# dnjulek/vapoursynth-zip

Hardware: AMD Instinct MI355X
Metric: frames/sec at 4K YUV420P16: Bilateral, BoxBlur, SSIMULACRA2 on 1/2/4/8 MI355X (higher is better)
Workload: dtype u16; 1 GPU; vszip.BoxBlur hradius=vradius=13, 3840x2160 YUV420P16, splitmix64 noise, HBM-resident; parallelism=frame-parallel x1, arena_candidates=5

## Files before the change

vapoursynth-zip_amd/csrc/boxblur_ct.hpp:

```cpp
#pragma once
#include <cmath>
#include <cstdlib>
#include <utility>

#include "plane_table.hpp"

namespace {

#ifndef VSZIP_ST_AUX
#define VSZIP_ST_AUX 2
#endif
#ifndef VSZIP_LD_AUX
#define VSZIP_LD_AUX 0
#endif
#ifndef VSZIP_ST8_AUX
#define VSZIP_ST8_AUX 0
#endif
#ifndef VSZIP_ST16_AUX
#define VSZIP_ST16_AUX 2
#endif
constexpr int kStoreAux = VSZIP_ST_AUX, kLoadAux = VSZIP_LD_AUX, kStoreAux8 = VSZIP_ST8_AUX, kStoreAux16 = VSZIP_ST16_AUX;
typedef uint32_t U32x4 __attribute__((ext_vector_type(4)));
typedef uint32_t U32x2 __attribute__((ext_vector_type(2)));

constexpr int kMaxPlanes = 48;
constexpr int PX = 8;

struct BBPlane {
    const void *src;
    void *dst;
    int sstride, dstride;
    int w, h;
    int block0;
    int ntx;
    int nbands;
    int nperiods;
    int cx0;
};

struct BBParams {
    BBPlane p[kMaxPlanes];
    int nplanes;
    int band_rows;
    int nblocks;
};

constexpr int kRingMaxPlanes = 192;
constexpr int kRingMaxBlocks = 8192;
struct RingParams {
    BBPlane p[kRingMaxPlanes];
    int nplanes;
    int nblocks;
    uint8_t plane_of_block[kRingMaxBlocks];
};

__device__ __forceinline__ int ct_tap_row(int k, int i, int radius, int ih) {
    const int dist_from_bottom = ih - 1 - i;
    if (k < radius) return (i < radius - k) ? min(radius - k - i, ih - 1) : (i - radius + k);
    return (dist_from_bottom < k - radius) ? (i - min(k - radius - dist_from_bottom, i)) : (i - radius + k);
}

template <typename T>
struct Raw8;
template <>
struct Raw8<uint16_t> {
    uint4 q;
};
template <>
struct Raw8<uint8_t> {
    uint2 q;
};

__device__ __forceinline__ void unpack8(const Raw8<uint16_t> &r, uint32_t v[PX]) {
    v[0] = r.q.x & 0xffffu; v[1] = r.q.x >> 16;
    v[2] = r.q.y & 0xffffu; v[3] = r.q.y >> 16;
    v[4] = r.q.z & 0xffffu; v[5] = r.q.z >> 16;
    v[6] = r.q.w & 0xffffu; v[7] = r.q.w >> 16;
}

__device__ __forceinline__ void unpack8(const Raw8<uint8_t> &r, uint32_t v[PX]) {
    v[0] = r.q.x & 0xffu; v[1] = (r.q.x >> 8) & 0xffu; v[2] = (r.q.x >> 16) & 0xffu; v[3] = r.q.x >> 24;
    v[4] = r.q.y & 0xffu; v[5] = (r.q.y >> 8) & 0xffu; v[6] = (r.q.y >> 16) & 0xffu; v[7] = r.q.y >> 24;
}

__device__ __forceinline__ void pack8(const uint32_t v[PX], Raw8<uint16_t> &r) {
    r.q.x = v[0] | (v[1] << 16);
    r.q.y = v[2] | (v[3] << 16);
    r.q.z = v[4] | (v[5] << 16);
    r.q.w = v[6] | (v[7] << 16);
// ... 133 lines not shown
    }

    const int ci = lane * PX;
#pragma unroll 1
    for (int i = y0; i < y1; ++i) {
        Raw8<T> an, sn;
        const bool more = i + 1 < y1;
        if (more) {
            const int n = i + 1;
            const int ar = (n + R < h) ? n + R : n - 1;
            const int sr = (n <= R) ? R - n + 1 : n - R - 1;
            an = load8<T>(src + (size_t)ar * pl.sstride, vx0, w, in_fast);
            sn = load8<T>(src + (size_t)sr * pl.sstride, vx0, w, in_fast);
        }

        uint32_t p[PX];
#pragma unroll
        for (int k = 0; k < PX; ++k) p[k] = __umulhi(col[k] + R, MAGIC);
#pragma unroll
        for (int k = 1; k < PX; ++k) p[k] += p[k - 1];
        const uint32_t incl = DPP ? wave_incl_scan_dpp(p[PX - 1]) : wave_incl_scan_shfl(p[PX - 1]);
        const uint32_t base = incl - p[PX - 1];
#pragma unroll
        for (int k = 0; k < PX; ++k) p[k] += base;
        *reinterpret_cast<uint4 *>(&P[ci]) = make_uint4(p[0], p[1], p[2], p[3]);
        *reinterpret_cast<uint4 *>(&P[ci + 4]) = make_uint4(p[4], p[5], p[6], p[7]);
        wave_lds_fence();

        if (is_out) {
            const uint32_t e0 = P[R] + P[R - 1];
            const uint32_t krow = 32768u + (uint32_t)(((uint64_t)e0 * INVLO) >> 16);
            uint32_t o[PX];
#pragma unroll
            for (int k = 0; k < PX; ++k) {
                const uint32_t e = P[ci + k + R] - P[ci + k - R - 1];
                o[k] = (uint32_t)(((uint64_t)e * INV2 + krow) >> 16);
            }
            store8<T>(dst + (size_t)i * pl.dstride, vx0, w, out_fast, o);
        }
        wave_lds_fence();

        if (more) {
            uint32_t a[PX], sb[PX];
            unpack8(an, a);
            unpack8(sn, sb);
#pragma unroll
            for (int k = 0; k < PX; ++k) col[k] += a[k] - sb[k];
        }
    }
}



template <int R, int SLOT_VGPRS = 4, int PXN = 8, int RV = R>
struct RingGeom {
    static constexpr int K = 2 * RV + 1;
    static constexpr int HL = ((R + 1 + PXN - 1) / PXN) * PXN;
    static constexpr int HR = ((R + PXN - 1) / PXN) * PXN;
#ifdef VSZIP_RING_OUT_LANES
    static constexpr int OUT_LANES = VSZIP_RING_OUT_LANES < 64 - HL / PXN - HR / PXN ? VSZIP_RING_OUT_LANES : 64 - HL / PXN - HR / PXN;
#else
    static constexpr int OUT_LANES = 64 - HL / PXN - HR / PXN;
#endif
    static constexpr int TWO = OUT_LANES * PXN;
    static constexpr int est_vgprs(int d) { return (2 * RV + 1 + d) * SLOT_VGPRS + (PXN == 16 ? 104 : 56); }
    static constexpr int tier(int v) { return v <= 128 ? 4 : (v <= 168 ? 3 : 2); }
    static constexpr int D3 = (2 * RV + 4) % 3 == 0 ? 3 : ((2 * RV + 6) % 3 == 0 ? 5 : 7);
#ifdef VSZIP_RING_D
    static constexpr int D = VSZIP_RING_D | 1;
    static constexpr int KL = (2 * RV + 1 + D) % 3 == 0 ? 3 : 2;
#else
    static constexpr bool SHALLOW = tier(est_vgprs(1)) > tier(est_vgprs(D3));
    static constexpr int D = SHALLOW ? 1 : D3;
    static constexpr int KL = SHALLOW ? 2 : 3;
#endif
    static constexpr int NR = 2 * RV + 1 + D;
#ifdef VSZIP_RING_WPE
    static constexpr int WPE = VSZIP_RING_WPE;
#else
    static constexpr int WPE = (SLOT_VGPRS == 2 && PXN == 8) ? (tier(est_vgprs(D)) > 3 ? 3 : tier(est_vgprs(D))) : tier(est_vgprs(D));
#endif
    static_assert(NR % KL == 0, "K-column ring must divide the period");
    static constexpr uint32_t MAGIC = K > 1 ? (uint32_t)(((1ull << 32) + K - 1) / K) : 0u;
};

template <typename T, int R, bool GENERAL, int PXN = 8, bool HONLY = false>
struct RingWave {
    static_assert(PXN == 8 || (PXN == 16 && sizeof(T) == 1 && !GENERAL), "16 pixels a lane: 8-bit planes, whole 16-pixel groups");
    static constexpr int RV = HONLY ? 0 : R;
    using G = RingGeom<R, (int)(sizeof(T) * PXN / 4), PXN, RV>;
    using RawT = RawN<T, PXN>;
    using Vec = decltype(RawT{}.q);
    static constexpr int NR = G::NR;
    static constexpr uint64_t INV = ((1ull << 32) + R) / (uint64_t)(2 * R + 1);
    static constexpr uint32_t INV2 = (uint32_t)(INV >> 16);

    RawT ring[NR];
    uint32_t col[PXN];
    uint32_t kcol;
    uint32_t kwgt;
    uint32_t kvo;
    uint32_t kn[G::KL], ko[G::KL];
    uint32_t kn_off, ko_off;
    uint32_t kr_prev;
    uint32_t *P;
    const char *srcb;
    char *dstb;
    uint32_t coff;
    uint32_t doff;
    uint32_t next_off;
    uint32_t out_off;
    uint32_t srow, drow;
    int w, h, lane, c0;
    bool rev, ld_ok, is_out, out_full;
    bool plain;
    __amdgpu_buffer_rsrc_t rs, rd;
    uint32_t sdoff;
    uint32_t psel;
    static constexpr uint32_t kOOB = 0xfffffff0u;

    __device__ __forceinline__ RawT fetch_off(uint32_t row_off) const {
        RawT t;
        if constexpr (sizeof(T) * PXN == 16) {
            const auto v = __builtin_amdgcn_raw_buffer_load_b128(rs, coff, row_off, sizeof(T) == 2 ? kLoadAux : 0);
            t.q = make_uint4(v[0], v[1], v[2], v[3]);
        } else {
            const auto v = __builtin_amdgcn_raw_buffer_load_b64(rs, coff, row_off, 0);
            t.q = make_uint2(v[0], v[1]);
        }
        return t;
    }
    __device__ __forceinline__ uint32_t fetch_px(uint32_t row_off) const {
        if constexpr (sizeof(T) == 2)
            return __builtin_amdgcn_raw_buffer_load_b16(rs, kvo, row_off, 0);
        else
            return __builtin_amdgcn_raw_buffer_load_b8(rs, kvo, row_off, 0);
    }
    __device__ __forceinline__ uint32_t krow_now() const {
        constexpr uint32_t INVLO = (uint32_t)(INV & 0xffffu);
        uint32_t v = __umul24(G::K > 1 ? __umulhi(kcol, G::MAGIC) : kcol, kwgt);
        v += (uint32_t)__builtin_amdgcn_update_dpp(0, (int)v, 0x111, 0xf, 0xf, false);
        v += (uint32_t)__builtin_amdgcn_update_dpp(0, (int)v, 0x112, 0xf, 0xf, false);
        v += (uint32_t)__builtin_amdgcn_update_dpp(0, (int)v, 0x114, 0xf, 0xf, false);
        v += (uint32_t)__builtin_amdgcn_update_dpp(0, (int)v, 0x118, 0xf, 0xf, false);
        uint32_t e0;
        if constexpr (R < 16) {
            e0 = (uint32_t)__builtin_amdgcn_readlane((int)v, 15);
        } else {
            v += (uint32_t)__builtin_amdgcn_update_dpp(0, (int)v, 0x142, 0xa, 0xf, false);
            e0 = (uint32_t)__builtin_amdgcn_readlane((int)v, 31);
        }
        return 32768u + (uint32_t)(((uint64_t)e0 * INVLO) >> 16);
    }

    __device__ __forceinline__ void fix_order(RawT &r) const {
        if constexpr (GENERAL) return;
        if constexpr (sizeof(T) * PXN == 16) {
            const uint4 o = r.q;
            r.q.x = __builtin_amdgcn_perm(o.w, o.x, psel);
            r.q.y = __builtin_amdgcn_perm(o.z, o.y, psel);
            r.q.z = __builtin_amdgcn_perm(o.y, o.z, psel);
            r.q.w = __builtin_amdgcn_perm(o.x, o.w, psel);
        } else {
            const uint2 o = r.q;
            r.q.x = __builtin_amdgcn_perm(o.y, o.x, psel);
            r.q.y = __builtin_amdgcn_perm(o.x, o.y, psel);
        }
    }
    __device__ __forceinline__ uint32_t row_off(int v) const {
        const int r = v < 0 ? -v : (v < h ? v : v - RV - 1);
        return (uint32_t)min(r, h - 1) * srow;
// ... 70 lines not shown
            } else if constexpr (PXN == 16) {
                uint32_t dw[4];
#pragma unroll
                for (int g = 0; g < 4; ++g) {
                    const uint32_t a0 = __builtin_amdgcn_perm(t[4 * g + 1], t[4 * g], 0x0c0c0602u);
                    const uint32_t a1 = __builtin_amdgcn_perm(t[4 * g + 3], t[4 * g + 2], 0x0c0c0602u);
                    dw[g] = a0 | (a1 << 16);
                }
                U32x4 v;
                v.x = dw[0];
                v.y = dw[1];
                v.z = dw[2];
                v.w = dw[3];
                __builtin_amdgcn_raw_buffer_store_b128(v, rd, vo, row_off_bytes, kStoreAux16);
            } else {
                U32x2 v;
                const uint32_t a0 = __builtin_amdgcn_perm(t[1], t[0], 0x0c0c0602u);
                const uint32_t a1 = __builtin_amdgcn_perm(t[3], t[2], 0x0c0c0602u);
                const uint32_t a2 = __builtin_amdgcn_perm(t[5], t[4], 0x0c0c0602u);
                const uint32_t a3 = __builtin_amdgcn_perm(t[7], t[6], 0x0c0c0602u);
                v.x = a0 | (a1 << 16);
                v.y = a2 | (a3 << 16);
                __builtin_amdgcn_raw_buffer_store_b64(v, rd, vo, row_off_bytes, kStoreAux8);
            }
        } else {
            T *q = reinterpret_cast<T *>(dstb + (row_off_bytes + doff));
            if (out_full) {
                if constexpr (sizeof(T) == 2) {
                    uint4 v;
                    v.x = __builtin_amdgcn_perm(t[1], t[0], 0x07060302u);
                    v.y = __builtin_amdgcn_perm(t[3], t[2], 0x07060302u);
                    v.z = __builtin_amdgcn_perm(t[5], t[4], 0x07060302u);
                    v.w = __builtin_amdgcn_perm(t[7], t[6], 0x07060302u);
                    *reinterpret_cast<uint4 *>(q) = v;
                } else {
                    uint2 v;
                    const uint32_t a0 = __builtin_amdgcn_perm(t[1], t[0], 0x0c0c0602u);
                    const uint32_t a1 = __builtin_amdgcn_perm(t[3], t[2], 0x0c0c0602u);
                    const uint32_t a2 = __builtin_amdgcn_perm(t[5], t[4], 0x0c0c0602u);
                    const uint32_t a3 = __builtin_amdgcn_perm(t[7], t[6], 0x0c0c0602u);
                    v.x = a0 | (a1 << 16);
                    v.y = a2 | (a3 << 16);
                    *reinterpret_cast<uint2 *>(q) = v;
                }
            } else {
#pragma unroll
                for (int k = 0; k < PXN; ++k)
                    if (c0 + k < w) q[k] = (T)(t[k] >> 16);
            }
        }
    }

    template <int S>
    __device__ __forceinline__ void step(int i, int y0) {
        uint32_t *Pa = P + (S & 1) * (64 * PXN);
        const uint32_t *Pb = P + ((S & 1) ^ 1) * (64 * PXN);
        __builtin_amdgcn_sched_barrier(0);

        uint32_t e[PXN];
        const bool have_prev = S > 0 || i > y0;
#ifdef VSZIP_DIAG_NO_HORIZONTAL
#pragma unroll
        for (int k = 0; k < PXN; ++k) e[k] = col[k];
#else
        if (!GENERAL || have_prev) window_sums(Pb, e);
#endif

        uint32_t p[PXN];
#pragma unroll
        for (int k = 0; k < PXN; ++k) {
            if constexpr (G::K == 1) {
                p[k] = col[k];
            } else if constexpr (sizeof(T) == 1) {
                constexpr uint32_t M19 = (uint32_t)(((1u << 19) + G::K - 1) / G::K);
                static_assert((uint64_t)(255u * G::K + RV) * (M19 * G::K - (1u << 19)) < (1u << 19), "8-bit divide-by-k shortcut must be exact");
                p[k] = __umul24(col[k], M19) >> 19;
            } else {
                p[k] = __umulhi(col[k], G::MAGIC);
            }
        }
        if constexpr (GENERAL) {
            const uint32_t m = ld_ok ? 0xffffffffu : 0u;
#pragma unroll
            for (int k = 0; k < PXN; ++k) p[k] &= m;
        }
#ifdef VSZIP_DIAG_NO_HORIZONTAL
        (void)Pa;
        kr_prev += p[0] + p[7];
#else
#pragma unroll
        for (int k = 1; k < PXN; ++k) p[k] += p[k - 1];
        const uint32_t incl = wave_incl_scan_dpp(p[PXN - 1]);
        const uint32_t base = incl - p[PXN - 1];
#pragma unroll
        for (int k = 0; k < PXN; ++k) Pa[k * 64 + lane] = p[k] + base;
#endif

        {
            constexpr int E = (S + 1 + 2 * RV) % NR;
            uint32_t a[PXN], sb[PXN];
            fix_order(ring[E]);
            unpackN(ring[E], a);
            unpackN(ring[S], sb);
#pragma unroll
            for (int k = 0; k < PXN; ++k) col[k] += a[k] - sb[k];
#ifdef VSZIP_DIAG_NO_LOAD
            if (next_off == 0xffffffffu) ring[S] = fetch_off(next_off);
#else
            ring[S] = fetch_off(next_off);
#endif

        }
        const uint32_t kr_cur = krow_now();
        {
            constexpr int J = S % G::KL;
            kcol += kn[J] - ko[J];
#ifndef VSZIP_DIAG_NO_KCOL
            kn[J] = fetch_px(kn_off);
            ko[J] = fetch_px(ko_off);
#endif

        }

        emit_row(e, out_off, kr_prev, have_prev);
        out_off += have_prev ? drow : 0u;
        kr_prev = kr_cur;
        if (plain) {
            next_off += srow;
            kn_off += srow;
            ko_off += srow;
        } else {
            next_off = row_off(i + 2 + RV + G::D);
            kn_off = row_off(i + 2 + RV + G::KL);
            ko_off = row_off(i + 1 - RV + G::KL);
        }
#ifndef VSZIP_DIAG_NO_FENCE
        wave_lds_fence();
#endif
    }

    template <int... S>
    __device__ __forceinline__ void period(int i0, int y0, std::integer_sequence<int, S...>) {
        (step<S>(i0 + S, y0), ...);
    }
};

template <typename T, int R, bool GENERAL, int PXN = 8, bool HONLY = false>
__global__ __launch_bounds__(64, (GENERAL ? 2 : RingGeom<R, (int)(sizeof(T) * PXN / 4), PXN, (HONLY ? 0 : R)>::WPE)) void boxblur_ct_ring_kernel(const RingParams prm) {
    using W = RingWave<T, R, GENERAL, PXN, HONLY>;
    using G = typename W::G;
    constexpr int RV = W::RV;
    static_assert(G::NR % 2 == 0 && G::NR <= 64, "ring period must be even and fit a wave");
    __shared__ __attribute__((aligned(16))) uint32_t P[2 * 64 * PXN];

    const int chunk = (prm.nblocks + 7) >> 3;
    const int b = (int)(blockIdx.x & 7) * chunk + (int)(blockIdx.x >> 3);
    if (b >= prm.nblocks) return;
    const int pi = prm.plane_of_block[b];
    const BBPlane pl = prm.p[pi];
    const int lb = b - pl.block0;
    const int tx = lb % pl.ntx;
    const int by = lb / pl.ntx;
    const int p0 = (int)((long)by * pl.nperiods / pl.nbands);
    const int p1 = (int)((long)(by + 1) * pl.nperiods / pl.nbands);
    const int band_rows = (p1 - p0) * G::NR;
    const int y0 = min(p0 * G::NR, pl.h - band_rows);
    const int w = pl.w;

    W st;
    st.P = P;
    st.w = w;
    st.h = pl.h;
    st.srow = (uint32_t)pl.sstride * (uint32_t)sizeof(T);
    st.drow = (uint32_t)pl.dstride * (uint32_t)sizeof(T);
    st.srcb = static_cast<const char *>(pl.src);
    st.dstb = static_cast<char *>(pl.dst);
    const int lane = threadIdx.x;
    st.lane = lane;
    const int vc0 = pl.cx0 + tx * G::TWO - G::HL + lane * PXN;
    st.c0 = vc0;
    st.is_out = lane >= G::HL / PXN && lane < G::HL / PXN + G::OUT_LANES && vc0 < w;
    st.doff = (uint32_t)(max(vc0, 0) * (int)sizeof(T));
    st.out_full = vc0 + PXN <= w;
    if constexpr (!GENERAL) {
        int g = vc0;
        st.rev = false;
        if (vc0 < 0) {
            g = -vc0 - PXN;
            st.rev = true;
        } else if (vc0 >= w) {
            g = 2 * w - vc0 - PXN;
            st.rev = true;
        }
        g = min(max(g, 0), w - PXN);
        st.coff = (uint32_t)(g * (int)sizeof(T));
        st.ld_ok = true;
    } else {
        st.rev = false;
        st.ld_ok = vc0 >= 0 && vc0 < w;
        st.coff = (uint32_t)(min(max(vc0, 0), ((w - 1) / PXN) * PXN) * (int)sizeof(T));
    }

    st.psel = st.rev ? (sizeof(T) == 2 ? 0x05040706u : 0x04050607u) : 0x03020100u;
    st.sdoff = st.is_out ? st.doff : W::kOOB;
    st.rs = __builtin_amdgcn_make_buffer_rsrc(const_cast<void *>(pl.src), 0, (int)((uint32_t)pl.h * st.srow), 0x00020000);
    st.rd = __builtin_amdgcn_make_buffer_rsrc(pl.dst, 0, (int)((uint32_t)pl.h * st.drow), 0x00020000);
    st.plain = (y0 - RV >= 0) && (y0 + band_rows + RV + G::D + 2 < pl.h);

    st.fill_all(y0, std::make_integer_sequence<int, G::NR>{});
#pragma unroll
    for (int k = 0; k < PXN; ++k) st.col[k] = RV;
    st.accum_all(std::make_integer_sequence<int, (int)G::K>{});
    {
        const int kc = min(lane, R);
        st.kvo = (uint32_t)(kc * (int)sizeof(T));
        st.kwgt = lane < R ? 2u : (lane == R ? 1u : 0u);
        uint32_t acc = RV;
#pragma unroll
        for (int k = 0; k < (int)G::K; ++k) acc += st.fetch_px(st.row_off(y0 - RV + k));
        st.kcol = acc;
#pragma unroll
        for (int j = 0; j < G::KL; ++j) {
            st.kn[j] = st.fetch_px(st.row_off(y0 + j + 1 + RV));
            st.ko[j] = st.fetch_px(st.row_off(y0 + j - RV));
        }
        st.kn_off = st.row_off(y0 + G::KL + 1 + RV);
        st.ko_off = st.row_off(y0 + G::KL - RV);
        st.kr_prev = 0;
    }
    st.next_off = st.row_off(y0 + 1 + RV + G::D);
    st.out_off = (uint32_t)y0 * st.drow;

    const int y1 = y0 + band_rows;
#pragma unroll 1
    for (int i0 = y0; i0 < y1; i0 += G::NR) st.period(i0, y0, std::make_integer_sequence<int, G::NR>{});
    {
        uint32_t e[PXN];
        st.window_sums(P + 64 * PXN, e);
        st.emit_row(e, st.out_off, st.kr_prev, true);
    }
}


template <typename T, int R>
int launch_ct_int(vszip_ctx *ctx, const vszip_plane *planes, int nplanes) {
    using G = CtGeom<R>;
    int done = 0;
    while (done < nplanes) {
        BBParams prm;
        const int n = std::min(kMaxPlanes, nplanes - done);
        prm.nplanes = n;
        long total_px = 0;
        for (int i = 0; i < n; ++i) total_px += (long)planes[done + i].w * planes[done + i].h;
        int band = 64;
        while (band > 16 && total_px / ((long)G::TWO * band) < 4096) band >>= 1;
        prm.band_rows = band;
        int blocks = 0;
        for (int i = 0; i < n; ++i) {
            const vszip_plane &s = planes[done + i];
            BBPlane &d = prm.p[i];
            d.src = s.src;
            d.dst = s.dst;
            d.sstride = (int)s.src_stride;
            d.dstride = (int)s.dst_stride;
            d.w = s.w;
            d.h = s.h;
            d.block0 = blocks;
            d.ntx = (s.w + G::TWO - 1) / G::TWO;
            d.nbands = (s.h + band - 1) / band;
            blocks += d.ntx * d.nbands;
        }
        if (ctx->scan_mode == 1)
            hipLaunchKernelGGL((boxblur_ct_int_kernel<T, R, false>), dim3(blocks), dim3(64), 0, ctx->stream, prm);
        else
            hipLaunchKernelGGL((boxblur_ct_int_kernel<T, R, true>), dim3(blocks), dim3(64), 0, ctx->stream, prm);
        VSZIP_HIP_CHECK(ctx, hipGetLastError());
        done += n;
    }
    return VSZIP_OK;
}

struct RingSpan {
    int cx0, ntx;
};

template <typename T, int R, int PXN, bool HONLY = false>
int ring_plan(const vszip_plane *planes, const RingSpan *spans, int n, double *waves_ret) {
    using G = typename RingWave<T, R, false, PXN, HONLY>::G;
    struct Geo {
        int h, ntx, count;
    };
    std::vector<Geo> geos;
    for (int i = 0; i < n; ++i) {
        bool found = false;
        for (Geo &g : geos)
            if (g.h == planes[i].h && g.ntx == spans[i].ntx) {
                ++g.count;
                found = true;
                break;
            }
        if (!found) geos.push_back({planes[i].h, spans[i].ntx, 1});
    }
        auto bands_for = [](int h, int P, int target) { return std::max((h % G::NR != 0 && P >= 2) ? 2 : 1, (P + target / 2) / target); };
        const double halo_p = (double)(G::K - 1 + G::D) / G::NR;
        const double slots = 256.0 * 4 * G::WPE;
        double waves_out = 0;
        auto cost_for = [&](int target) {
            double work = 0, waves = 0, max_len = 0;
            for (const Geo &g : geos) {
                const int P = (g.h + G::NR - 1) / G::NR;
                const int nb = bands_for(g.h, P, target);
                const double ntx = (double)g.ntx * g.count;
                work += ntx * (P + nb * halo_p);
                waves += ntx * nb;
                max_len = std::max(max_len, (double)((P + nb - 1) / nb) + halo_p);
            }
            waves_out = waves;
            const double gens = std::ceil(waves / slots);
            const double eff = std::min(1.0, work / (slots * gens * max_len));
            return std::max(work / slots * (1.0 + 0.3 * (1.0 - eff)), 0.3 * max_len);
        };
        int target = 1;
        double best = cost_for(1);
        const double min_waves = std::min(0.6 * slots, waves_out);
        for (int t = 2; t <= 96; ++t) {
            const double c = cost_for(t);
            if (waves_out >= min_waves && c < best) {
                best = c;
                target = t;
            }
        }
        *waves_ret = (cost_for(target), waves_out);
        return target;
}


template <typename T, int R, int PXN, bool GEN, bool HONLY = false>
int launch_ct_ring_spans(vszip_ctx *ctx, const vszip_plane *all_planes, const RingSpan *all_spans, int nall) {
    using G = typename RingWave<T, R, false, PXN, HONLY>::G;
    std::vector<vszip_plane> planes_v;
    std::vector<RingSpan> spans_v;
    for (int i = 0; i < nall; ++i)
        if (all_spans[i].ntx > 0) {
            planes_v.push_back(all_planes[i]);
            spans_v.push_back(all_spans[i]);
        }
    const vszip_plane *planes = planes_v.data();
    const RingSpan *spans = spans_v.data();
    const int nplanes = (int)planes_v.size();
    int done = 0;
    while (done < nplanes) {
        RingParams prm;
        const int n = std::min(kRingMaxPlanes, nplanes - done);
        auto bands_for = [](int h, int P, int target) { return std::max((h % G::NR != 0 && P >= 2) ? 2 : 1, (P + target / 2) / target); };
        double waves_out = 0;
        int target = ring_plan<T, R, PXN, HONLY>(planes + done, spans + done, n, &waves_out);
        if (ctx->opt.ring_periods > 0) target = ctx->opt.ring_periods;
#ifdef VSZIP_RING_PERIODS_FIXED
        target = VSZIP_RING_PERIODS_FIXED;
#endif
#ifdef VSZIP_RING_PLAN_DEBUG
        fprintf(stderr, "ring plan PX%d GEN%d r=%d: n=%d target=%d waves=%.0f slots=%d NR=%d | plane0 %dx%d ntx=%d\n", PXN, (int)GEN, R, n, target, waves_out, 256 * 4 * G::WPE, G::NR,
                planes[done].w, planes[done].h, spans[done].ntx);
#endif
        VSZIP_HIP_CHECK(ctx, hipSetDevice(ctx->device));
        int blocks = 0, fit = n;
        for (int i = 0; i < n; ++i) {
            const vszip_plane &s = planes[done + i];
            BBPlane &d = prm.p[i];
            d.src = s.src;
            d.dst = s.dst;
            d.sstride = (int)s.src_stride;
            d.dstride = (int)s.dst_stride;
            d.w = s.w;
            d.h = s.h;
            d.nperiods = (s.h + G::NR - 1) / G::NR;
            d.nbands = bands_for(s.h, d.nperiods, target);
            d.ntx = spans[done + i].ntx;
            d.cx0 = spans[done + i].cx0;
            d.block0 = blocks;
            if (blocks + d.ntx * d.nbands > kRingMaxBlocks) {
                if (i == 0) return vszip_set_error(ctx, VSZIP_ERR_ARG, "BoxBlur: launch table overflow (%d blocks)", blocks + d.ntx * d.nbands);
                fit = i;
                break;
            }
            for (int k = 0; k < d.ntx * d.nbands; ++k) prm.plane_of_block[blocks + k] = (uint8_t)i;
            blocks += d.ntx * d.nbands;
        }
        prm.nplanes = fit;
        prm.nblocks = blocks;
        const dim3 grid(((blocks + 7) / 8) * 8);
        {
            vszip_probe_scope probe(ctx);
            hipLaunchKernelGGL((boxblur_ct_ring_kernel<T, R, GEN, PXN, HONLY>), grid, dim3(64), 0, ctx->stream, prm);
        }
        VSZIP_HIP_CHECK(ctx, hipGetLastError());
        done += fit;
    }
    return VSZIP_OK;
}

template <typename T>
bool ring_ok(const vszip_plane *planes, int nplanes) {
    constexpr uintptr_t VB = sizeof(T) * PX;
    for (int i = 0; i < nplanes; ++i) {
        const vszip_plane &p = planes[i];
        if ((reinterpret_cast<uintptr_t>(p.src) | reinterpret_cast<uintptr_t>(p.dst) | (uintptr_t)(p.src_stride * sizeof(T)) | (uintptr_t)(p.dst_stride * sizeof(T))) & (VB - 1)) return false;
        if (p.src_stride < ((p.w + PX - 1) / PX) * PX) return false;
        if (p.src_stride < 24) return false;
        if (p.h < 2 * 22 + 1 + 8) return false;
        if ((uint64_t)p.src_stride * p.h * sizeof(T) >= (1ull << 32) || (uint64_t)p.dst_stride * p.h * sizeof(T) >= (1ull << 32)) return false;
    }
    return true;
}

constexpr int kRing16MaxR = 19;
template <typename T, int R, bool HONLY = false>
bool ring16_ok(const vszip_ctx *ctx, const vszip_plane *planes, int nplanes) {
    if (sizeof(T) != 1 || ctx->opt.ct_u8_px8) return false;
    using G16 = RingGeom<R, 4, 16, (HONLY ? 0 : R)>;
    using G8 = RingGeom<R, 2, 8, (HONLY ? 0 : R)>;
    double px = 0, t16 = 0, t8 = 0;
    for (int i = 0; i < nplanes; ++i) {
        const vszip_plane &p = planes[i];
        if (p.w < 32) return false;
        if ((reinterpret_cast<uintptr_t>(p.src) | reinterpret_cast<uintptr_t>(p.dst) | (uintptr_t)p.src_stride | (uintptr_t)p.dst_stride) & 15) return false;
        px += (double)p.w * p.h;
        t16 += (double)((p.w + G16::TWO - 1) / G16::TWO) * G16::TWO * p.h;
        t8 += (double)((p.w + G8::TWO - 1) / G8::TWO) * G8::TWO * p.h;
    }
    if (R >= 8 && px / t16 < 0.93 * (px / t8)) return false;
    if (R >= 8) {
        const int n = std::min(nplanes, kRingMaxPlanes);
        std::vector<RingSpan> s16(n), s8(n);
        for (int i = 0; i < n; ++i) {
            s16[i] = {0, (planes[i].w + G16::TWO - 1) / G16::TWO};
            s8[i] = {0, (planes[i].w + G8::TWO - 1) / G8::TWO};
        }
        double w16 = 0, w8 = 0;
        ring_plan<T, R, 16, HONLY>(planes, s16.data(), n, &w16);
        ring_plan<T, R, 8, HONLY>(planes, s8.data(), n, &w8);
        const double f16 = w16 / (256.0 * 4 * G16::WPE), f8 = w8 / (256.0 * 4 * G8::WPE);
        if (f16 < 0.8 && f8 > f16 + 0.05) return false;
    }
    return true;
}

template <typename T, int R, int PXF, bool HONLY = false>
int run_ct_ring(vszip_ctx *ctx, const vszip_plane *planes, int nplanes) {
    using GF = typename RingWave<T, R, false, PXF, HONLY>::G;
    using GG = typename RingWave<T, R, true, 8, HONLY>::G;
    std::vector<RingSpan> fast(nplanes), rest(nplanes);
    bool any_rest = false, any_fast = false;
    for (int i = 0; i < nplanes; ++i) {
        const int w = planes[i].w;
        if (w % PXF == 0) {
            fast[i] = {0, (w + GF::TWO - 1) / GF::TWO};
            rest[i] = {0, 0};
        } else {
            const int room = w + GF::HL - 64 * PXF;
            const int nsafe = room >= 0 ? room / GF::TWO + 1 : 0;
            fast[i] = {0, nsafe};
            const int x = nsafe * GF::TWO;
            rest[i] = {x, (w - x + GG::TWO - 1) / GG::TWO};
        }
        any_fast = any_fast || fast[i].ntx > 0;
        any_rest = any_rest || rest[i].ntx > 0;
    }
    if (any_fast) {
        const int rc = launch_ct_ring_spans<T, R, PXF, false, HONLY>(ctx, planes, fast.data(), nplanes);
        if (rc != VSZIP_OK) return rc;
    }
    if (any_rest) return launch_ct_ring_spans<T, R, 8, true, HONLY>(ctx, planes, rest.data(), nplanes);
    return VSZIP_OK;
// ... 42 lines not shown
```

Baseline: 112,000 frames/s.

## Split ring-blur bands at arbitrary row boundaries instead of whole periods

Bands of rows for the ring box-blur kernel can now end at any row instead of being rounded to a multiple of the ring period. Each wave can leave the period loop early once it reaches its last row, and a separate tail emit covers the final row. The planner now chooses a band count per reference height, capped so bands keep a minimum row count, with the aim of balancing waves across slots and cutting the overlapping rows that came from period rounding. A few radius/type combinations keep the old period-aligned path, and the host table fill switches to memset.

```diff
diff --git a/vapoursynth-zip_amd/csrc/boxblur_ct.hpp b/vapoursynth-zip_amd/csrc/boxblur_ct.hpp
--- a/vapoursynth-zip_amd/csrc/boxblur_ct.hpp
+++ b/vapoursynth-zip_amd/csrc/boxblur_ct.hpp
@@ -1,6 +1,7 @@
 #pragma once
 #include <cmath>
 #include <cstdlib>
+#include <cstring>
 #include <utility>
 
 #include "plane_table.hpp"
@@ -34,7 +35,6 @@
     int block0;
     int ntx;
     int nbands;
-    int nperiods;
     int cx0;
 };
 
@@ -306,8 +306,12 @@
     static constexpr uint32_t MAGIC = K > 1 ? (uint32_t)(((1ull << 32) + K - 1) / K) : 0u;
 };
 
+template <typename T, int R, bool GENERAL, int PXN, bool HONLY>
+constexpr bool kRingRowCut = HONLY || !((sizeof(T) == 2 && !GENERAL && (R == 5 || R == 6)) || (sizeof(T) == 2 && GENERAL && R >= 14) || (sizeof(T) == 1 && PXN == 16 && R == 17));
+
 template <typename T, int R, bool GENERAL, int PXN = 8, bool HONLY = false>
 struct RingWave {
+    static constexpr bool ROWCUT = kRingRowCut<T, R, GENERAL, PXN, HONLY>;
     static_assert(PXN == 8 || (PXN == 16 && sizeof(T) == 1 && !GENERAL), "16 pixels a lane: 8-bit planes, whole 16-pixel groups");
     static constexpr int RV = HONLY ? 0 : R;
     using G = RingGeom<R, (int)(sizeof(T) * PXN / 4), PXN, RV>;
@@ -515,13 +519,13 @@
     }
 
     template <int S>
-    __device__ __forceinline__ void step(int i, int y0) {
+    __device__ __forceinline__ void step(int i, int y0, int y1) {
         uint32_t *Pa = P + (S & 1) * (64 * PXN);
         const uint32_t *Pb = P + ((S & 1) ^ 1) * (64 * PXN);
         __builtin_amdgcn_sched_barrier(0);
 
         uint32_t e[PXN];
-        const bool have_prev = S > 0 || i > y0;
+        const bool have_prev = (S > 0 || i > y0) && (ROWCUT || i <= y1);
 #ifdef VSZIP_DIAG_NO_HORIZONTAL
 #pragma unroll
         for (int k = 0; k < PXN; ++k) e[k] = col[k];
@@ -603,8 +607,12 @@
     }
 
     template <int... S>
-    __device__ __forceinline__ void period(int i0, int y0, std::integer_sequence<int, S...>) {
-        (step<S>(i0 + S, y0), ...);
+    __device__ __forceinline__ bool period(int i0, int y0, int y1, std::integer_sequence<int, S...>) {
+        return ((step<S>(i0 + S, y0, y1), __builtin_expect(i0 + S + 1 >= y1, 0)) || ...);
+    }
+    template <int... S>
+    __device__ __forceinline__ void whole_period(int i0, int y0, int y1, std::integer_sequence<int, S...>) {
+        (step<S>(i0 + S, y0, y1), ...);
     }
 };
 
@@ -624,10 +632,16 @@
     const int lb = b - pl.block0;
     const int tx = lb % pl.ntx;
     const int by = lb / pl.ntx;
-    const int p0 = (int)((long)by * pl.nperiods / pl.nbands);
-    const int p1 = (int)((long)(by + 1) * pl.nperiods / pl.nbands);
-    const int band_rows = (p1 - p0) * G::NR;
-    const int y0 = min(p0 * G::NR, pl.h - band_rows);
+    int y0, y1, y_run;
+    if constexpr (W::ROWCUT) {
+        y0 = (int)((long)by * pl.h / pl.nbands);
+        y_run = y1 = (int)((long)(by + 1) * pl.h / pl.nbands);
+    } else {
+        const int nper = (pl.h + G::NR - 1) / G::NR;
+        y0 = (int)((long)by * nper / pl.nbands) * G::NR;
+        y_run = (int)((long)(by + 1) * nper / pl.nbands) * G::NR;
+        y1 = min(y_run, pl.h);
+    }
     const int w = pl.w;
 
     W st;
@@ -668,7 +682,7 @@
     st.sdoff = st.is_out ? st.doff : W::kOOB;
     st.rs = __builtin_amdgcn_make_buffer_rsrc(const_cast<void *>(pl.src), 0, (int)((uint32_t)pl.h * st.srow), 0x00020000);
     st.rd = __builtin_amdgcn_make_buffer_rsrc(pl.dst, 0, (int)((uint32_t)pl.h * st.drow), 0x00020000);
-    st.plain = (y0 - RV >= 0) && (y0 + band_rows + RV + G::D + 2 < pl.h);
+    st.plain = (y0 - RV >= 0) && (y_run + RV + G::D + 2 < pl.h);
 
     st.fill_all(y0, std::make_integer_sequence<int, G::NR>{});
 #pragma unroll
@@ -694,13 +708,22 @@
     st.next_off = st.row_off(y0 + 1 + RV + G::D);
     st.out_off = (uint32_t)y0 * st.drow;
 
-    const int y1 = y0 + band_rows;
+    if constexpr (W::ROWCUT) {
 #pragma unroll 1
-    for (int i0 = y0; i0 < y1; i0 += G::NR) st.period(i0, y0, std::make_integer_sequence<int, G::NR>{});
-    {
+        for (int i0 = y0; !st.period(i0, y0, y1, std::make_integer_sequence<int, G::NR>{}); i0 += G::NR) {
+        }
+        uint32_t e[PXN];
+        if ((y1 - y0) & 1)
+            st.window_sums(P, e);
+        else
+            st.window_sums(P + 64 * PXN, e);
+        st.emit_row(e, st.out_off, st.kr_prev, true);
+    } else {
+#pragma unroll 1
+        for (int i0 = y0; i0 < y1; i0 += G::NR) st.whole_period(i0, y0, y1, std::make_integer_sequence<int, G::NR>{});
         uint32_t e[PXN];
         st.window_sums(P + 64 * PXN, e);
-        st.emit_row(e, st.out_off, st.kr_prev, true);
+        st.emit_row(e, st.out_off, st.kr_prev, y1 == y_run);
     }
 }
 
@@ -747,15 +770,39 @@
     int cx0, ntx;
 };
 
+#ifndef VSZIP_RING_MIN_BAND_ROWS
+#define VSZIP_RING_MIN_BAND_ROWS 14
+#endif
+constexpr int kRingMinBandRows = VSZIP_RING_MIN_BAND_ROWS;
+struct RingPlan {
+    int href, nb;
+    int period;
+    int target;
+};
+inline int ring_bands(RingPlan plan, int h) {
+    if (plan.period) {
+        const int P = (h + plan.period - 1) / plan.period;
+        return std::max((h % plan.period != 0 && P >= 2) ? 2 : 1, (P + plan.target / 2) / plan.target);
+    }
+    const int nb = (int)(((long)h * plan.nb + plan.href / 2) / plan.href);
+    return std::max(1, std::min(nb, h / kRingMinBandRows));
+}
+inline RingPlan ring_plan_rows(RingPlan plan, int rows, int NR) {
+    if (plan.period) return {plan.href, plan.nb, plan.period, std::max(1, rows / NR)};
+    return {plan.href, std::max(1, (plan.href + rows / 2) / rows), 0, 0};
+}
+
 template <typename T, int R, int PXN, bool HONLY = false>
-int ring_plan(const vszip_plane *planes, const RingSpan *spans, int n, double *waves_ret) {
+RingPlan ring_plan(const vszip_plane *planes, const RingSpan *spans, int n, double *waves_ret, bool row_cut = kRingRowCut<T, R, false, PXN, HONLY>) {
     using G = typename RingWave<T, R, false, PXN, HONLY>::G;
     struct Geo {
         int h, ntx, count;
     };
     std::vector<Geo> geos;
+    int href = 1;
     for (int i = 0; i < n; ++i) {
         bool found = false;
+        href = std::max(href, planes[i].h);
         for (Geo &g : geos)
             if (g.h == planes[i].h && g.ntx == spans[i].ntx) {
                 ++g.count;
@@ -764,37 +811,38 @@
             }
         if (!found) geos.push_back({planes[i].h, spans[i].ntx, 1});
     }
-        auto bands_for = [](int h, int P, int target) { return std::max((h % G::NR != 0 && P >= 2) ? 2 : 1, (P + target / 2) / target); };
-        const double halo_p = (double)(G::K - 1 + G::D) / G::NR;
-        const double slots = 256.0 * 4 * G::WPE;
-        double waves_out = 0;
-        auto cost_for = [&](int target) {
-            double work = 0, waves = 0, max_len = 0;
-            for (const Geo &g : geos) {
-                const int P = (g.h + G::NR - 1) / G::NR;
-                const int nb = bands_for(g.h, P, target);
-                const double ntx = (double)g.ntx * g.count;
-                work += ntx * (P + nb * halo_p);
-                waves += ntx * nb;
-                max_len = std::max(max_len, (double)((P + nb - 1) / nb) + halo_p);
-            }
-            waves_out = waves;
-            const double gens = std::ceil(waves / slots);
-            const double eff = std::min(1.0, work / (slots * gens * max_len));
-            return std::max(work / slots * (1.0 + 0.3 * (1.0 - eff)), 0.3 * max_len);
-        };
-        int target = 1;
-        double best = cost_for(1);
-        const double min_waves = std::min(0.6 * slots, waves_out);
-        for (int t = 2; t <= 96; ++t) {
-            const double c = cost_for(t);
-            if (waves_out >= min_waves && c < best) {
-                best = c;
-                target = t;
-            }
-        }
-        *waves_ret = (cost_for(target), waves_out);
-        return target;
+    const int halo = G::K - 1 + G::D;
+    const double slots = 256.0 * 4 * G::WPE;
+    double waves_out = 0;
+    auto cost_for = [&](int nbref) {
+        double work = 0, waves = 0, max_len = 0;
+        for (const Geo &g : geos) {
+            const int nb = ring_bands(row_cut ? RingPlan{href, nbref, 0, 0} : RingPlan{href, 0, G::NR, nbref}, g.h);
+            const double ntx = (double)g.ntx * g.count;
+            const int P = (g.h + G::NR - 1) / G::NR;
+            const int rows = row_cut ? g.h : P * G::NR, longest = row_cut ? (g.h + nb - 1) / nb : (P + nb - 1) / nb * G::NR;
+            work += ntx * (rows + nb * halo);
+            waves += ntx * nb;
+            max_len = std::max(max_len, (double)(longest + halo));
+        }
+        waves_out = waves;
+        const double gens = std::ceil(waves / slots);
+        const double eff = std::min(1.0, work / (slots * gens * max_len));
+        return std::max(work / slots * (1.0 + 0.3 * (1.0 - eff)), 0.3 * max_len);
+    };
+    const int first = row_cut ? std::max(1, href / kRingMinBandRows) : 1, last = row_cut ? 1 : 96, dir = row_cut ? -1 : 1;
+    int nbref = first;
+    double best = cost_for(nbref);
+    const double min_waves = std::min(0.6 * slots, waves_out);
+    for (int t = first + dir; t != last + dir; t += dir) {
+        const double c = cost_for(t);
+        if (waves_out >= min_waves && c < best) {
+            best = c;
+            nbref = t;
+        }
+    }
+    *waves_ret = (cost_for(nbref), waves_out);
+    return row_cut ? RingPlan{href, nbref, 0, 0} : RingPlan{href, 0, G::NR, nbref};
 }
 
 
@@ -815,16 +863,20 @@
     while (done < nplanes) {
         RingParams prm;
         const int n = std::min(kRingMaxPlanes, nplanes - done);
-        auto bands_for = [](int h, int P, int target) { return std::max((h % G::NR != 0 && P >= 2) ? 2 : 1, (P + target / 2) / target); };
         double waves_out = 0;
-        int target = ring_plan<T, R, PXN, HONLY>(planes + done, spans + done, n, &waves_out);
-        if (ctx->opt.ring_periods > 0) target = ctx->opt.ring_periods;
+        RingPlan plan = ring_plan<T, R, PXN, HONLY>(planes + done, spans + done, n, &waves_out, kRingRowCut<T, R, GEN, PXN, HONLY>);
+        if (ctx->opt.ring_periods > 0) plan = ring_plan_rows(plan, ctx->opt.ring_periods * G::NR, G::NR);
 #ifdef VSZIP_RING_PERIODS_FIXED
-        target = VSZIP_RING_PERIODS_FIXED;
+        plan = ring_plan_rows(plan, VSZIP_RING_PERIODS_FIXED * G::NR, G::NR);
 #endif
 #ifdef VSZIP_RING_PLAN_DEBUG
-        fprintf(stderr, "ring plan PX%d GEN%d r=%d: n=%d target=%d waves=%.0f slots=%d NR=%d | plane0 %dx%d ntx=%d\n", PXN, (int)GEN, R, n, target, waves_out, 256 * 4 * G::WPE, G::NR,
-                planes[done].w, planes[done].h, spans[done].ntx);
+        {
+            const vszip_plane &f = planes[done], &l = planes[done + n - 1];
+            const int bf = ring_bands(plan, f.h), bl = ring_bands(plan, l.h);
+            fprintf(stderr, "ring plan PX%d GEN%d r=%d: %d planes, %.0f waves on %d slots, NR=%d | first plane %dx%d: %d tiles x %d bands of %d-%d rows | last plane %dx%d: %d tiles x %d bands of %d-%d rows\n",
+                    PXN, (int)GEN, R, n, waves_out, 256 * 4 * G::WPE, G::NR, f.w, f.h, spans[done].ntx, bf, f.h / bf, (f.h + bf - 1) / bf, l.w, l.h, spans[done + n - 1].ntx, bl, l.h / bl,
+                    (l.h + bl - 1) / bl);
+        }
 #endif
         VSZIP_HIP_CHECK(ctx, hipSetDevice(ctx->device));
         int blocks = 0, fit = n;
@@ -837,8 +889,7 @@
             d.dstride = (int)s.dst_stride;
             d.w = s.w;
             d.h = s.h;
-            d.nperiods = (s.h + G::NR - 1) / G::NR;
-            d.nbands = bands_for(s.h, d.nperiods, target);
+            d.nbands = ring_bands(plan, s.h);
             d.ntx = spans[done + i].ntx;
             d.cx0 = spans[done + i].cx0;
             d.block0 = blocks;
@@ -847,7 +898,7 @@
                 fit = i;
                 break;
             }
-            for (int k = 0; k < d.ntx * d.nbands; ++k) prm.plane_of_block[blocks + k] = (uint8_t)i;
+            memset(prm.plane_of_block + blocks, i, (size_t)d.ntx * d.nbands);
             blocks += d.ntx * d.nbands;
         }
         prm.nplanes = fit;
```

After: 113,100 frames/s (median of 6 runs). Within noise of the previous version (+1.0%).

## Stream 16-bit ring rows through an LDS queue via buffer-load-to-LDS DMA

Applied to the files above, without the earlier changes.

For 16-bit planes with radius up to 13, the ring kernel now prefetches incoming rows and the K-column pixels into an LDS queue using buffer_load_dwordx4 with the lds modifier, in place of per-step register loads. Each step waits on vmcnt so that QD rows stay in flight, then reads the new row from LDS. The K-column vertical sums come from an LDS ring instead of per-pixel scalar loads, and the register ring depth drops to D=1. This is meant to cut VGPR pressure and load latency on the critical path, at the cost of more LDS per workgroup, inline asm that changes m0 and exec, and possible occupancy limits.

```diff
diff --git a/vapoursynth-zip_amd/csrc/boxblur_ct.hpp b/vapoursynth-zip_amd/csrc/boxblur_ct.hpp
--- a/vapoursynth-zip_amd/csrc/boxblur_ct.hpp
+++ b/vapoursynth-zip_amd/csrc/boxblur_ct.hpp
@@ -274,7 +274,50 @@
 
 
 
-template <int R, int SLOT_VGPRS = 4, int PXN = 8, int RV = R>
+#ifndef VSZIP_RING_QD
+#define VSZIP_RING_QD 2
+#endif
+#ifndef VSZIP_RING_QD_HI
+#define VSZIP_RING_QD_HI 0
+#endif
+constexpr int kRingQueueMaxR = 13;
+template <int R, int SLOT_VGPRS, int PXN, int RV, int QDEPTH>
+struct RingGeom;
+template <int R, int Q>
+constexpr int ring_queue_fit() {
+    if constexpr (Q < 2)
+        return 0;
+    else if constexpr (RingGeom<R, 4, 8, R, Q>::FITS)
+        return Q;
+    else
+        return ring_queue_fit<R, Q - 1>();
+}
+template <typename T, int R>
+constexpr int ring_queue_depth() {
+    if constexpr (sizeof(T) == 2)
+        return ring_queue_fit<R, (R <= kRingQueueMaxR ? VSZIP_RING_QD : VSZIP_RING_QD_HI)>();
+    else
+        return 0;
+}
+
+__device__ __forceinline__ void ring_dma16(__amdgpu_buffer_rsrc_t rs, uint32_t lds_byte, uint32_t voff, uint32_t soff) {
+    uint32_t keep;
+    asm volatile("s_mov_b32 %0, m0\n\ts_mov_b32 m0, %1\n\ts_nop 0\n\tbuffer_load_dwordx4 %2, %3, %4 offen lds\n\ts_mov_b32 m0, %0"
+                 : "=&s"(keep)
+                 : "s"(lds_byte), "v"(voff), "s"(rs), "s"(soff)
+                 : "memory");
+}
+template <int LANES>
+__device__ __forceinline__ void ring_dma16_first(__amdgpu_buffer_rsrc_t rs, uint32_t lds_byte, uint32_t voff, uint32_t soff) {
+    uint32_t keep;
+    uint64_t keep_exec;
+    asm volatile("s_mov_b32 %0, m0\n\ts_mov_b64 %1, exec\n\ts_mov_b32 m0, %2\n\ts_mov_b64 exec, %6\n\tbuffer_load_dwordx4 %3, %4, %5 offen lds\n\ts_mov_b64 exec, %1\n\ts_mov_b32 m0, %0"
+                 : "=&s"(keep), "=&s"(keep_exec)
+                 : "s"(lds_byte), "v"(voff), "s"(rs), "s"(soff), "n"((1 << LANES) - 1)
+                 : "memory");
+}
+
+template <int R, int SLOT_VGPRS, int PXN, int RV, int QDEPTH>
 struct RingGeom {
     static constexpr int K = 2 * RV + 1;
     static constexpr int HL = ((R + 1 + PXN - 1) / PXN) * PXN;
@@ -288,14 +331,21 @@
     static constexpr int est_vgprs(int d) { return (2 * RV + 1 + d) * SLOT_VGPRS + (PXN == 16 ? 104 : 56); }
     static constexpr int tier(int v) { return v <= 128 ? 4 : (v <= 168 ? 3 : 2); }
     static constexpr int D3 = (2 * RV + 4) % 3 == 0 ? 3 : ((2 * RV + 6) % 3 == 0 ? 5 : 7);
+    static constexpr int QD = QDEPTH;
+    static_assert(QD == 0 || QD >= 2, "the row queue is read one step after it is refilled");
+    static constexpr int KB = ((R + 1) * (16 / PXN) + 15) / 16 * 16;
+    static constexpr int KQ = 2 * RV + 2 + QD;
 #ifdef VSZIP_RING_D
-    static constexpr int D = VSZIP_RING_D | 1;
+    static constexpr int D = QD > 0 ? 1 : (VSZIP_RING_D | 1);
     static constexpr int KL = (2 * RV + 1 + D) % 3 == 0 ? 3 : 2;
 #else
-    static constexpr bool SHALLOW = tier(est_vgprs(1)) > tier(est_vgprs(D3));
+    static constexpr bool SHALLOW = QD > 0 || tier(est_vgprs(1)) > tier(est_vgprs(D3));
     static constexpr int D = SHALLOW ? 1 : D3;
     static constexpr int KL = SHALLOW ? 2 : 3;
 #endif
+    static constexpr int AHEAD = QD > 0 ? QD : D;
+    static constexpr int HALO_ROWS = QD > 0 ? 2 * RV : 2 * RV + D;
+    static constexpr int LDS_BYTES = 2 * 64 * PXN * 4 + (QD > 0 ? QD * 1024 + KQ * KB : 0);
     static constexpr int NR = 2 * RV + 1 + D;
 #ifdef VSZIP_RING_WPE
     static constexpr int WPE = VSZIP_RING_WPE;
@@ -303,6 +353,7 @@
     static constexpr int WPE = (SLOT_VGPRS == 2 && PXN == 8) ? (tier(est_vgprs(D)) > 3 ? 3 : tier(est_vgprs(D))) : tier(est_vgprs(D));
 #endif
     static_assert(NR % KL == 0, "K-column ring must divide the period");
+    static constexpr bool FITS = 4 * WPE * ((LDS_BYTES + 1279) / 1280 * 1280) <= 160 * 1024;
     static constexpr uint32_t MAGIC = K > 1 ? (uint32_t)(((1ull << 32) + K - 1) / K) : 0u;
 };
 
@@ -310,7 +361,9 @@
 struct RingWave {
     static_assert(PXN == 8 || (PXN == 16 && sizeof(T) == 1 && !GENERAL), "16 pixels a lane: 8-bit planes, whole 16-pixel groups");
     static constexpr int RV = HONLY ? 0 : R;
-    using G = RingGeom<R, (int)(sizeof(T) * PXN / 4), PXN, RV>;
+    static constexpr int QD = (!GENERAL && !HONLY && sizeof(T) * PXN == 16) ? ring_queue_depth<T, R>() : 0;
+    using G = RingGeom<R, (int)(sizeof(T) * PXN / 4), PXN, RV, QD>;
+    static_assert(QD == 0 || G::FITS, "row queue too deep for this many workgroups a CU");
     using RawT = RawN<T, PXN>;
     using Vec = decltype(RawT{}.q);
     static constexpr int NR = G::NR;
@@ -339,6 +392,10 @@
     __amdgpu_buffer_rsrc_t rs, rd;
     uint32_t sdoff;
     uint32_t psel;
+    uint32_t q_slot, k_new, k_in, k_out;
+    uint32_t q_lds, k_lds;
+    uint32_t kdoff;
+    int yend;
     static constexpr uint32_t kOOB = 0xfffffff0u;
 
     __device__ __forceinline__ RawT fetch_off(uint32_t row_off) const {
@@ -520,6 +577,18 @@
         const uint32_t *Pb = P + ((S & 1) ^ 1) * (64 * PXN);
         __builtin_amdgcn_sched_barrier(0);
 
+        uint32_t k_enter = 0, k_leave = 0;
+        if constexpr (QD > 0) {
+            asm volatile("s_waitcnt vmcnt(%0) lgkmcnt(0)" ::"n"(3 * QD - 4) : "memory");
+            __builtin_amdgcn_wave_barrier();
+            const bool wanted = i + QD + 2 <= yend;
+            ring_dma16(rs, q_lds + q_slot * 1024u, wanted ? coff : kOOB, next_off);
+            ring_dma16_first<G::KB / 16>(rs, k_lds + k_new * (uint32_t)G::KB, wanted ? kdoff : kOOB, next_off);
+            const T *kq = reinterpret_cast<const T *>(P + 2 * 64 * PXN + QD * 256);
+            k_enter = kq[k_in * (G::KB / sizeof(T)) + kvo / sizeof(T)];
+            k_leave = kq[k_out * (G::KB / sizeof(T)) + kvo / sizeof(T)];
+        }
+
         uint32_t e[PXN];
         const bool have_prev = S > 0 || i > y0;
 #ifdef VSZIP_DIAG_NO_HORIZONTAL
@@ -567,15 +636,25 @@
             unpackN(ring[S], sb);
 #pragma unroll
             for (int k = 0; k < PXN; ++k) col[k] += a[k] - sb[k];
+            if constexpr (QD > 0) {
+                q_slot = q_slot + 1 == QD ? 0 : q_slot + 1;
+                ring[S].q = *reinterpret_cast<const uint4 *>(P + 2 * 64 * PXN + q_slot * 256 + lane * 4);
+            } else {
 #ifdef VSZIP_DIAG_NO_LOAD
-            if (next_off == 0xffffffffu) ring[S] = fetch_off(next_off);
+                if (next_off == 0xffffffffu) ring[S] = fetch_off(next_off);
 #else
-            ring[S] = fetch_off(next_off);
-#endif
+                ring[S] = fetch_off(next_off);
+#endif
+            }
 
         }
         const uint32_t kr_cur = krow_now();
-        {
+        if constexpr (QD > 0) {
+            kcol += k_enter - k_leave;
+            k_new = k_new + 1 == G::KQ ? 0 : k_new + 1;
+            k_in = k_in + 1 == G::KQ ? 0 : k_in + 1;
+            k_out = k_out + 1 == G::KQ ? 0 : k_out + 1;
+        } else {
             constexpr int J = S % G::KL;
             kcol += kn[J] - ko[J];
 #ifndef VSZIP_DIAG_NO_KCOL
@@ -590,12 +669,16 @@
         kr_prev = kr_cur;
         if (plain) {
             next_off += srow;
-            kn_off += srow;
-            ko_off += srow;
+            if constexpr (QD == 0) {
+                kn_off += srow;
+                ko_off += srow;
+            }
         } else {
-            next_off = row_off(i + 2 + RV + G::D);
-            kn_off = row_off(i + 2 + RV + G::KL);
-            ko_off = row_off(i + 1 - RV + G::KL);
+            next_off = row_off(i + 2 + RV + G::AHEAD);
+            if constexpr (QD == 0) {
+                kn_off = row_off(i + 2 + RV + G::KL);
+                ko_off = row_off(i + 1 - RV + G::KL);
+            }
         }
 #ifndef VSZIP_DIAG_NO_FENCE
         wave_lds_fence();
@@ -609,12 +692,12 @@
 };
 
 template <typename T, int R, bool GENERAL, int PXN = 8, bool HONLY = false>
-__global__ __launch_bounds__(64, (GENERAL ? 2 : RingGeom<R, (int)(sizeof(T) * PXN / 4), PXN, (HONLY ? 0 : R)>::WPE)) void boxblur_ct_ring_kernel(const RingParams prm) {
+__global__ __launch_bounds__(64, (GENERAL ? 2 : RingWave<T, R, GENERAL, PXN, HONLY>::G::WPE)) void boxblur_ct_ring_kernel(const RingParams prm) {
     using W = RingWave<T, R, GENERAL, PXN, HONLY>;
     using G = typename W::G;
     constexpr int RV = W::RV;
     static_assert(G::NR % 2 == 0 && G::NR <= 64, "ring period must be even and fit a wave");
-    __shared__ __attribute__((aligned(16))) uint32_t P[2 * 64 * PXN];
+    __shared__ __attribute__((aligned(16))) uint32_t P[G::LDS_BYTES / 4];
 
     const int chunk = (prm.nblocks + 7) >> 3;
     const int b = (int)(blockIdx.x & 7) * chunk + (int)(blockIdx.x >> 3);
@@ -668,7 +751,10 @@
     st.sdoff = st.is_out ? st.doff : W::kOOB;
     st.rs = __builtin_amdgcn_make_buffer_rsrc(const_cast<void *>(pl.src), 0, (int)((uint32_t)pl.h * st.srow), 0x00020000);
     st.rd = __builtin_amdgcn_make_buffer_rsrc(pl.dst, 0, (int)((uint32_t)pl.h * st.drow), 0x00020000);
-    st.plain = (y0 - RV >= 0) && (y0 + band_rows + RV + G::D + 2 < pl.h);
+    if constexpr (G::QD > 0)
+        st.plain = (y0 - RV >= 0) && (y0 + band_rows + RV <= pl.h);
+    else
+        st.plain = (y0 - RV >= 0) && (y0 + band_rows + RV + G::D + 2 < pl.h);
 
     st.fill_all(y0, std::make_integer_sequence<int, G::NR>{});
 #pragma unroll
@@ -682,19 +768,40 @@
 #pragma unroll
         for (int k = 0; k < (int)G::K; ++k) acc += st.fetch_px(st.row_off(y0 - RV + k));
         st.kcol = acc;
-#pragma unroll
-        for (int j = 0; j < G::KL; ++j) {
-            st.kn[j] = st.fetch_px(st.row_off(y0 + j + 1 + RV));
-            st.ko[j] = st.fetch_px(st.row_off(y0 + j - RV));
-        }
-        st.kn_off = st.row_off(y0 + G::KL + 1 + RV);
-        st.ko_off = st.row_off(y0 + G::KL - RV);
+        if constexpr (G::QD == 0) {
+#pragma unroll
+            for (int j = 0; j < G::KL; ++j) {
+                st.kn[j] = st.fetch_px(st.row_off(y0 + j + 1 + RV));
+                st.ko[j] = st.fetch_px(st.row_off(y0 + j - RV));
+            }
+            st.kn_off = st.row_off(y0 + G::KL + 1 + RV);
+            st.ko_off = st.row_off(y0 + G::KL - RV);
+        }
         st.kr_prev = 0;
     }
-    st.next_off = st.row_off(y0 + 1 + RV + G::D);
+    st.next_off = st.row_off(y0 + 1 + RV + G::AHEAD);
     st.out_off = (uint32_t)y0 * st.drow;
 
     const int y1 = y0 + band_rows;
+    if constexpr (G::QD > 0) {
+        constexpr int QD = G::QD;
+        st.yend = y1;
+        st.q_lds = (uint32_t)(uintptr_t)P + 2 * 64 * PXN * 4;
+        st.k_lds = st.q_lds + QD * 1024;
+        st.kdoff = (uint32_t)lane * 16u;
+#pragma unroll 1
+        for (int u = 0; u <= 2 * RV + QD; ++u) {
+            const uint32_t off = st.row_off(y0 - RV + u);
+            ring_dma16_first<G::KB / 16>(st.rs, st.k_lds + (uint32_t)u * G::KB, st.kdoff, off);
+            if (u >= 2 * RV + 2) ring_dma16(st.rs, st.q_lds + (uint32_t)(u % QD) * 1024u, st.coff, off);
+        }
+        st.q_slot = (2 * RV + 1) % QD;
+        st.k_new = 2 * RV + 1 + QD;
+        st.k_in = 2 * RV + 1;
+        st.k_out = 0;
+        asm volatile("s_waitcnt vmcnt(0)" ::: "memory");
+        __builtin_amdgcn_wave_barrier();
+    }
 #pragma unroll 1
     for (int i0 = y0; i0 < y1; i0 += G::NR) st.period(i0, y0, std::make_integer_sequence<int, G::NR>{});
     {
@@ -702,6 +809,7 @@
         st.window_sums(P + 64 * PXN, e);
         st.emit_row(e, st.out_off, st.kr_prev, true);
     }
+    if constexpr (G::QD > 0) asm volatile("s_waitcnt vmcnt(0)" ::: "memory");
 }
 
 
@@ -747,9 +855,9 @@
     int cx0, ntx;
 };
 
-template <typename T, int R, int PXN, bool HONLY = false>
+template <typename T, int R, int PXN, bool HONLY = false, bool GEN = false>
 int ring_plan(const vszip_plane *planes, const RingSpan *spans, int n, double *waves_ret) {
-    using G = typename RingWave<T, R, false, PXN, HONLY>::G;
+    using G = typename RingWave<T, R, GEN, PXN, HONLY>::G;
     struct Geo {
         int h, ntx, count;
     };
@@ -765,7 +873,7 @@
         if (!found) geos.push_back({planes[i].h, spans[i].ntx, 1});
     }
         auto bands_for = [](int h, int P, int target) { return std::max((h % G::NR != 0 && P >= 2) ? 2 : 1, (P + target / 2) / target); };
-        const double halo_p = (double)(G::K - 1 + G::D) / G::NR;
+        const double halo_p = (double)G::HALO_ROWS / G::NR;
         const double slots = 256.0 * 4 * G::WPE;
         double waves_out = 0;
         auto cost_for = [&](int target) {
@@ -800,7 +908,7 @@
 
 template <typename T, int R, int PXN, bool GEN, bool HONLY = false>
 int launch_ct_ring_spans(vszip_ctx *ctx, const vszip_plane *all_planes, const RingSpan *all_spans, int nall) {
-    using G = typename RingWave<T, R, false, PXN, HONLY>::G;
+    using G = typename RingWave<T, R, GEN, PXN, HONLY>::G;
     std::vector<vszip_plane> planes_v;
     std::vector<RingSpan> spans_v;
     for (int i = 0; i < nall; ++i)
@@ -817,7 +925,7 @@
         const int n = std::min(kRingMaxPlanes, nplanes - done);
         auto bands_for = [](int h, int P, int target) { return std::max((h % G::NR != 0 && P >= 2) ? 2 : 1, (P + target / 2) / target); };
         double waves_out = 0;
-        int target = ring_plan<T, R, PXN, HONLY>(planes + done, spans + done, n, &waves_out);
+        int target = ring_plan<T, R, PXN, HONLY, GEN>(planes + done, spans + done, n, &waves_out);
         if (ctx->opt.ring_periods > 0) target = ctx->opt.ring_periods;
 #ifdef VSZIP_RING_PERIODS_FIXED
         target = VSZIP_RING_PERIODS_FIXED;
@@ -881,8 +989,8 @@
 template <typename T, int R, bool HONLY = false>
 bool ring16_ok(const vszip_ctx *ctx, const vszip_plane *planes, int nplanes) {
     if (sizeof(T) != 1 || ctx->opt.ct_u8_px8) return false;
-    using G16 = RingGeom<R, 4, 16, (HONLY ? 0 : R)>;
-    using G8 = RingGeom<R, 2, 8, (HONLY ? 0 : R)>;
+    using G16 = RingGeom<R, 4, 16, (HONLY ? 0 : R), 0>;
+    using G8 = RingGeom<R, 2, 8, (HONLY ? 0 : R), 0>;
     double px = 0, t16 = 0, t8 = 0;
     for (int i = 0; i < nplanes; ++i) {
         const vszip_plane &p = planes[i];
```

Result: faster. 111,900 frames/s before, 114,500 frames/s after, median of 6 (+2.3%).
